# muelea/tuch

Hardware: AMD Instinct MI355X
Metric: SMPLify-DC fit iters/sec at batch 64 (higher is better)
Workload: dtype f32; 1 GPU; configs[1] extended to the full stage-2 step: batch=64/GPU SMPL forward + contact_fitting_loss (L_P/L_C push/pull, winding inside test, segment filter, r2r) + backward + Adam, V=6890 F=13776, float32; bodies_per_gpu=64, global_batch=64, launch=hipGraph replay of the whole step

## Files before the change

include/tuch_amd.h:

```cpp
#ifndef TUCH_AMD_H
#define TUCH_AMD_H

#include <stddef.h>
#include <stdint.h>

#ifdef __cplusplus
extern "C" {
#endif

const char* tuch_last_error(void);
int tuch_abi_version(void);

typedef struct tuch_contact_model tuch_contact_model;


int tuch_batch_pairwise_dist(const float* x, const float* y, int B, int Nx, int Ny, int squared,
                             float* P, void* stream);

int tuch_batch_pairwise_dist_bwd(const float* x, const float* y, const float* grad_P, int B, int Nx, int Ny,
                                 int squared, float* grad_x, float* grad_y, void* stream);

int tuch_solid_angles_bwd(const float* points, const float* triangles, const float* grad_out, const float* grad_w,
                          int B, int Q, int F, float* grad_points, float* grad_triangles, void* stream);

// ... 103 lines not shown
int tuch_contact_model_get_option(const tuch_contact_model* model, const char* name, int* value);
int tuch_contact_model_canary_hits(const tuch_contact_model* model, int* hits_host, int reset);
int tuch_contact_model_canary_selftest(const tuch_contact_model* model, void* workspace, size_t workspace_bytes, void* stream);
const uint64_t* tuch_contact_model_mask_bits(const tuch_contact_model* model);
const uint64_t* tuch_contact_model_tree_mask_bits(const tuch_contact_model* model);
int tuch_contact_model_info(const tuch_contact_model* model, int* V, int* F, int* num_segments,
                            int* seg_q_total, int* num_pairs);
int tuch_contact_model_strips(const tuch_contact_model* model, int* stream_len, int* num_strips,
                              int32_t* vidx_host, float* sign_host);

int tuch_winding_tree_work(const tuch_contact_model* model, const float* verts, int B, void* workspace,
                           size_t workspace_bytes, unsigned long long* out_host, void* stream);

int tuch_ray_work(const tuch_contact_model* model, const float* verts, int B, void* workspace,
                  size_t workspace_bytes, unsigned long long* out_host, void* stream);
int tuch_contact_model_tree_order(const tuch_contact_model* model, int32_t* qperm_host, int32_t* face_leaf_host);

size_t tuch_v2v_model_workspace_bytes(const tuch_contact_model* model, int B);
size_t tuch_v2v_hint_bytes(const tuch_contact_model* model, int B);
enum { TUCH_V2V_LEAVE_ROOM = 1, TUCH_V2V_NEAR_FINAL = 2 };
int tuch_v2v_min_model(const tuch_contact_model* model, const float* verts, int B, float* min_d2, int32_t* argmin,
                       void* hint_inout, void* workspace, size_t workspace_bytes, int flags, void* zero, size_t zero_bytes,
                       void* stream);

typedef struct tuch_cluster_tree tuch_cluster_tree;
int tuch_cluster_tree_build(int V, int F, const int32_t* faces, int leaf_faces, tuch_cluster_tree** out);
void tuch_cluster_tree_free(tuch_cluster_tree* tree);
int tuch_cluster_tree_info(const tuch_cluster_tree* tree, int* num_nodes, int* exact_len, int* stream_len,
                           int* num_qblocks, int* num_frontiers, int* frontier_total);
int tuch_cluster_tree_export(const tuch_cluster_tree* tree, int32_t* nodes, int32_t* vidx, float* sign,
// ... 128 lines not shown
```

tuch_amd/_C.py:

```python
from __future__ import annotations

import contextlib
import ctypes
import os
from ctypes import POINTER, c_char_p, c_float, c_int, c_size_t, c_uint, c_void_p

import torch

_HERE = os.path.dirname(os.path.abspath(__file__))
LIB_PATH = os.environ.get('TUCH_AMD_LIB') or os.path.join(_HERE, 'libtuch_amd.so')
_lib = None

ABI_VERSION = 2

_SIGNATURES = {
    'tuch_last_error': (c_char_p, []),
    'tuch_abi_version': (c_int, []),
    'tuch_batch_pairwise_dist': (c_int, [c_void_p, c_void_p, c_int, c_int, c_int, c_int, c_void_p, c_void_p]),
    'tuch_batch_pairwise_dist_bwd': (c_int, [c_void_p, c_void_p, c_void_p, c_int, c_int, c_int, c_int, c_void_p, c_void_p,
                                             c_void_p]),
    'tuch_solid_angles_bwd': (c_int, [c_void_p, c_void_p, c_void_p, c_void_p, c_int, c_int, c_int, c_void_p, c_void_p, c_void_p]),
    'tuch_solid_angles': (c_int, [c_void_p, c_void_p, c_int, c_int, c_int, c_void_p, c_void_p]),
    'tuch_gather_triangles': (c_int, [c_void_p, c_void_p, c_int, c_int, c_int, c_void_p, c_void_p]),
    'tuch_winding_workspace_bytes': (c_size_t, [c_int, c_int, c_int]),
# ... 56 lines not shown
    'tuch_estimate_translation': (c_int, [c_void_p, c_void_p, c_void_p, c_int, c_int, c_float, c_float, c_void_p, c_void_p]),
    'tuch_rotmat_to_angle_axis': (c_int, [c_void_p, c_int, c_int, c_void_p, c_void_p]),
    'tuch_winding_tree_work': (c_int, [c_void_p, c_void_p, c_int, c_void_p, c_size_t, c_void_p, c_void_p]),
    'tuch_hd_model_create': (c_int, [POINTER(c_void_p), c_void_p, c_int, c_void_p, c_void_p, c_void_p]),
    'tuch_hd_model_create_k': (c_int, [POINTER(c_void_p), c_void_p, c_int, c_int, c_void_p, c_void_p, c_void_p]),
    'tuch_hd_model_destroy': (None, [c_void_p]),
    'tuch_hd_model_info': (c_int, [c_void_p, POINTER(c_int), c_void_p]),
    'tuch_hd_contact_saved_bytes': (c_size_t, [c_void_p, c_int]),
    'tuch_hd_contact_workspace_bytes': (c_size_t, [c_void_p, c_int]),
    'tuch_hd_contact_fwd': (c_int, [c_void_p] * 6 + [c_int, c_float, c_float, c_void_p, c_void_p, c_size_t, c_void_p, c_size_t,
                                    c_void_p]),
    'tuch_hd_contact_bwd': (c_int, [c_void_p, c_void_p, c_void_p, c_int, c_void_p, c_void_p, c_size_t, c_void_p]),
    'tuch_hd_contact_selection': (c_int, [c_void_p, c_void_p, c_int, c_void_p, c_void_p]),
    'tuch_hd_contact_details': (c_int, [c_void_p, c_void_p, c_int, c_void_p, c_void_p]),
    'tuch_ray_work': (c_int, [c_void_p, c_void_p, c_int, c_void_p, c_size_t, c_void_p, c_void_p]),
    'tuch_contact_model_tree_order': (c_int, [c_void_p, c_void_p, c_void_p]),
    'tuch_v2v_model_workspace_bytes': (c_size_t, [c_void_p, c_int]),
    'tuch_v2v_hint_bytes': (c_size_t, [c_void_p, c_int]),
    'tuch_v2v_min_model': (c_int, [c_void_p, c_void_p, c_int, c_void_p, c_void_p, c_void_p, c_void_p, c_size_t, c_int,
                                   c_void_p, c_size_t, c_void_p]),
    'tuch_exterior_workspace_bytes': (c_size_t, [c_void_p, c_int]),
    'tuch_exterior_flags': (c_int, [c_void_p, c_void_p, c_int, c_int, c_float, c_void_p, c_void_p, c_void_p,
                                    c_void_p, c_void_p, c_size_t, c_void_p]),
    'tuch_winding_points_workspace_bytes': (c_size_t, [c_void_p, c_int, c_int]),
    'tuch_winding_points': (c_int, [c_void_p, c_void_p, c_void_p, c_void_p, c_int, c_int, c_float, c_void_p, c_void_p,
                                    c_void_p, c_size_t, c_void_p]),
    'tuch_closest_point_workspace_bytes': (c_size_t, [c_void_p, c_int, c_int]),
    'tuch_closest_point': (c_int, [c_void_p, c_void_p, c_void_p, c_void_p, c_int, c_int, c_void_p, c_void_p, c_void_p,
                                   c_void_p, c_size_t, c_void_p]),
    'tuch_closest_point_bwd': (c_int, [c_void_p] * 6 + [c_int, c_int] + [c_void_p] * 4),
# ... 106 lines not shown
```

tuch_amd/csrc/model.h:

```cpp
#pragma once
#include "common.h"
#include <vector>

enum { kNodeCapOff, kNodeCapLen, kNodeExactOff, kNodeExactLen, kNodeSkip, kNodeChild0, kNodeChild1, kNodeFaces, kNodeWords };
struct tuch_rows { int first, count; };
struct tuch_cluster_tree {
    int V = 0, F = 0, num_nodes = 0, exact_len = 0, stream_len = 0, num_qblocks = 0, num_heights = 0;
    std::vector<int32_t> nodes;
    std::vector<int32_t> vidx;
    std::vector<float> sign;
    std::vector<int32_t> qperm;
    std::vector<int32_t> height_off, height_nodes;
    std::vector<int32_t> frontier_off, frontier_nodes;
    std::vector<int32_t> launch_order;
    std::vector<int32_t> ancestors;
    std::vector<int32_t> rows;
    std::vector<int32_t> face_leaf;

    int node(int i, int field) const { return nodes[(size_t)i * kNodeWords + field]; }
    int skip(int i) const { return node(i, kNodeSkip); }
    int child0(int i) const { return node(i, kNodeChild0); }
    int child1(int i) const { return node(i, kNodeChild1); }
    bool is_leaf(int i) const { return child0(i) < 0; }
    int num_faces(int i) const { return node(i, kNodeFaces); }
// ... 4 lines not shown
};

bool tuch_cluster_tree_build_impl(int V, int F, const int32_t* faces, int leaf_faces, tuch_cluster_tree& t);
void tuch_build_strips(const int32_t* faces, int F, std::vector<int32_t>& vidx, std::vector<float>& sign,
                       int* num_strips);

struct tuch_contact_model;

struct tuch_options {
    int winding_ray = 1;
    int winding_tree = 1;
    int winding_strips = 1;
    int tree_waves = 32768;
    int ray_pair_cap = 16;
    int ray_waves = 32768;
    int v2v_tree = 1;
    int v2v_waves = 0;
    int v2v_flat = 2;
    int v2v_pairs = 24;
    int v2v_lds = -1;
    int seg_splits = 16;
    int seg_assist = 1;
    int seg_fused = 1;
    int canary = 0;
    int hd_search = 1;
    int hd_search_waves = 4;
    int hd_overlap = 1;
};
void tuch_options_from_env(tuch_options* o);

// ... 6 lines not shown
size_t tuch_ray_workspace_bytes(const tuch_contact_model* m, int B, int Q);
int tuch_ray_exterior_verts(const tuch_contact_model* m, const float* verts, int B, float thresh, uint8_t* exterior,
                            float* w, void* workspace, hipStream_t s, unsigned long long* stats_host,
                            uint8_t* exterior_copy = nullptr);
const int32_t* tuch_ray_segment_counts(const tuch_contact_model* m, int B, const void* workspace);
void tuch_ray_segment_prepare(const tuch_contact_model* m, const float* verts, const float* caps, int assisted, int B,
                              float* seg_entries, hipStream_t s);
bool tuch_ray_segment_fused_available(const tuch_contact_model* m);
int tuch_ray_segment_flags_one(const tuch_contact_model* m, const float* verts, const uint8_t* body_flags,
                               const int32_t* leaf_counts, int B, float thresh, uint8_t* exterior, hipStream_t s);
int tuch_ray_segment_flags(const tuch_contact_model* m, const float* verts, const float* caps, const int32_t* seg_count,
                           const int32_t* seg_list, const int32_t* leaf_counts, int B, int nsplit, float thresh, float* seg_tris,
                           int32_t* seg_partial, float* seg_w, uint8_t* seg_ext, uint8_t* exterior, hipStream_t s);
int tuch_ray_exterior_points(const tuch_contact_model* m, const float* verts, const float* points, const int32_t* counts,
                             int B, int Q, float thresh, uint8_t* exterior, float* w, void* workspace, hipStream_t s);

int tuch_v2v_min_indexed_seeded(const float* points, const int32_t* vertex_ids, const int32_t* offsets,
                                const int32_t* counts, const float* seed_best, const int32_t* seed_arg,
                                const int32_t* all_masked_arg, const uint64_t* geomask_bits, int B, int V,
                                int max_points_per_body, float* min_d2, int32_t* argmin, void* workspace, hipStream_t s);
extern "C" size_t tuch_v2v_min_indexed_workspace_bytes(int B, int max_points_per_body);
size_t tuch_hd_search_workspace_bytes(int B, int max_points_per_body);
int tuch_hd_search(const float* points, const int32_t* vertex_ids, const int32_t* offsets, const int32_t* counts,
                   const int32_t* all_masked_arg, const uint64_t* geomask_bits, int B, int V, int max_points_per_body,
                   float* min_d2, int32_t* argmin, void* workspace, hipStream_t s, int waves);
extern "C" size_t tuch_winding_points_workspace_bytes(const tuch_contact_model* m, int B, int Q);
extern "C" int tuch_winding_points(const tuch_contact_model* m, const float* verts, const float* points,
                                   const int32_t* counts, int B, int Q, float thresh, float* w,
                                   uint8_t* exterior, void* workspace, size_t workspace_bytes, void* stream);

// ... 73 lines not shown
```

tuch_amd/csrc/model.hip:

```cpp
#include "model.h"
#include <stdarg.h>
#include <stdio.h>
#include <stdlib.h>
#include <string.h>
#include <algorithm>
#include <vector>
#include <unordered_map>

extern "C" int tuch_geomask_words(int V);

namespace {

struct Segments {
    int count, num_caps;
    const int32_t *q_off, *q_vidx, *f_off, *faces;
};

struct SegmentLists {
    std::vector<int32_t> link_off{0}, links;
    std::vector<int32_t> ray_off{0}, ray_ent;
    std::vector<int32_t> elem_mask;
};

void debug_note(const char* fmt, ...)
// ... 431 lines not shown
        build_leaf_assist_tables(m, tree, faces, sg, lists);
    }
    if (num_regions > 0) build_region_tables(m, geomask, num_regions, region_off, region_vidx, num_pairs, pairs);
    if (!tree.sign.empty()) build_sign_words(m, tree, lists.elem_mask);
    const int rc = m->tables.rc;
    *out = rc == TUCH_OK ? m : nullptr;
    if (rc != TUCH_OK) tuch_contact_model_destroy(m);
    return rc;
}

namespace {
struct OptionName { const char* name; int tuch_options::*field; };
const OptionName kOptions[] = {
    {"winding_ray", &tuch_options::winding_ray}, {"winding_tree", &tuch_options::winding_tree},
    {"winding_strips", &tuch_options::winding_strips}, {"tree_waves", &tuch_options::tree_waves},
    {"ray_pair_cap", &tuch_options::ray_pair_cap}, {"ray_waves", &tuch_options::ray_waves},
    {"v2v_tree", &tuch_options::v2v_tree}, {"v2v_flat", &tuch_options::v2v_flat}, {"v2v_pairs", &tuch_options::v2v_pairs}, {"v2v_waves", &tuch_options::v2v_waves}, {"v2v_lds", &tuch_options::v2v_lds},
    {"seg_splits", &tuch_options::seg_splits}, {"seg_assist", &tuch_options::seg_assist}, {"seg_fused", &tuch_options::seg_fused},
    {"canary", &tuch_options::canary}, {"hd_search", &tuch_options::hd_search}, {"hd_search_waves", &tuch_options::hd_search_waves}, {"hd_overlap", &tuch_options::hd_overlap},
};
}

void tuch_options_from_env(tuch_options* o)
{
    for (const OptionName& k : kOptions) {
        char env[64] = "TUCH_";
        size_t n = strlen(env);
        for (const char* c = k.name; *c && n + 1 < sizeof(env); ++c) env[n++] = (char)toupper((unsigned char)*c);
        env[n] = 0;
        const char* e = getenv(env);
        if (e && *e) o->*(k.field) = atoi(e);
// ... 82 lines not shown
```

tuch_amd/csrc/ray_winding.hip:

```cpp
#include "common.h"
#include "model.h"
#include "workspace.h"
#include "tree_device.h"
#include <stdlib.h>

#pragma clang fp contract(off)

namespace {

constexpr float kPi = 3.14159265358979323846f;
constexpr int kBlock = 256;
constexpr int kRayQueries = 64;
constexpr float kShearX = 0.3217f, kShearY = 0.4331f;
constexpr float kFanX = 0.8191f, kFanY = 0.3467f, kFanZ = 0.4571f;
constexpr int kSlabs = 9;
constexpr int kSlabStride = 10;
constexpr int kNearSlabs = 13;

struct RayElem { float x, y, z, sign; };

__device__ __forceinline__ float shear_x(float x, float z) { return __builtin_fmaf(-kShearX, z, x); }
__device__ __forceinline__ float shear_y(float y, float z) { return __builtin_fmaf(-kShearY, z, y); }

__global__ __launch_bounds__(kBlock) void ray_stream_kernel(
// ... 94 lines not shown
        for (int p = Lexact + (int)threadIdx.x; p < T; p += kBoundsBlock)
            boxes[(size_t)b * T + p] = make_float4(__builtin_inff(), -__builtin_inff(), __builtin_inff(), -__builtin_inff());
    auto posed = [&](int p) {
        RayElem e;
        if (kPose) {
            const float* c = verts + ((size_t)b * V + vidx[p]) * 3;
            e.x = shear_x(c[0], c[2]); e.y = shear_y(c[1], c[2]); e.z = c[2]; e.sign = sign[p];
        } else {
            e = st[p];
        }
        return e;
    };
    float lo[kSlabs], nhi[kSlabs];
#pragma unroll
    for (int k = 0; k < kSlabs; ++k) { lo[k] = 3.0e38f; nhi[k] = 3.0e38f; }
    for (int p = sub; p < len; p += 16) {
        const RayElem e = posed(off + p);
        if (kPose) stream_out[(size_t)b * T + off + p] = e;
        boxes[(size_t)b * T + off + p] = ray_elem_box(posed(off + max(p - 2, 0)), posed(off + max(p - 1, 0)), e);
        float pr[kSlabs];
        slab_project(e.x, e.y, e.z, pr);
#pragma unroll
        for (int k = 0; k < kSlabs; ++k) { lo[k] = fminf(lo[k], pr[k]); nhi[k] = fminf(nhi[k], -pr[k]); }
    }
#pragma unroll
    for (int k = 0; k < kSlabs; ++k) { lo[k] = row_min(lo[k]); nhi[k] = row_min(nhi[k]); }
    if (real && sub == 0) {
        const int L = height_off[1] - height_off[0], leaf = i - height_off[0];
        float lo_p[kSlabs], hi_p[kSlabs];
#pragma unroll
        for (int k = 0; k < kSlabs; ++k) {
            const float hi = -nhi[k];
            const float pad = 4e-7f * fmaxf(fabsf(lo[k]), fabsf(hi)) + 1e-9f;
            lo_p[k] = lo[k] - pad;
            hi_p[k] = hi + pad;
        }
        float c[3];
        if (kPose) {
// ... 438 lines not shown
    }
    const int total_pairs = sp[kTilesBlock - 1], total_tiles = st[kTilesBlock - 1];
    const bool overflow = total_pairs > cap || total_tiles > max_tiles;
    if (t == 0) body[b] = RayBody{overflow ? fallback_tiles : total_tiles, overflow ? 1 : 0};
    if (overflow) return;
    int off = sp[t] - pairs, tile = st[t] - ntile;
    RayTile* out = tiles + (size_t)b * max_tiles;
    for (int l = l0; l < l1; ++l) {
        leaf_off[(size_t)b * num_leaves + l] = off;
        const TreeNode nd = nodes[leaf_nodes[l]];
        for (int k = 0; k < cnt[l]; k += 64) out[tile++] = RayTile{nd.ex_off, nd.ex_len, off + k, min(64, cnt[l] - k)};
        off += cnt[l];
    }
}

__global__ __launch_bounds__(64) void ray_fill_kernel(
    const RayEntry* __restrict__ lists, const int32_t* __restrict__ list_len, const RayBody* __restrict__ body,
    const int32_t* __restrict__ leaf_off, int num_leaves, int qblocks, int cap, int32_t* __restrict__ leaf_fill,
    int32_t* __restrict__ pairs)
{
    const int qb = blockIdx.x, b = blockIdx.y, lane = threadIdx.x;
    if (body[b].overflow) return;
    const int cnt = list_len[(size_t)b * qblocks + qb];
    const RayEntry* list = lists + ((size_t)b * qblocks + qb) * num_leaves;
    int32_t* out = pairs + (size_t)b * cap;
    for (int base = 0; base < cnt; base += 64) {
        const int j = base + lane;
        RayEntry e = RayEntry{0, 0, 0u, 0u};
        int dst = 0;
        if (j < cnt) {
            e = list[j];
            const int n = __builtin_popcount(e.mask_lo) + __builtin_popcount(e.mask_hi);
            dst = leaf_off[(size_t)b * num_leaves + e.leaf] + atomicAdd(&leaf_fill[(size_t)b * num_leaves + e.leaf], n);
        }
        const int m = min(64, cnt - base);
        for (int k = 0; k < m; ++k) {
            const uint32_t lo = __builtin_amdgcn_readlane(e.mask_lo, k), hi = __builtin_amdgcn_readlane(e.mask_hi, k);
            const int d = __builtin_amdgcn_readlane(dst, k);
            const unsigned long long mask = ((unsigned long long)hi << 32) | lo;
            if ((mask >> lane) & 1ull)
                out[d + __builtin_popcountll(mask & ((1ull << lane) - 1ull))] = qb * kRayQueries + lane;
        }
    }
}

constexpr int kTilesFillBlock = 64, kFillSplit = 64, kFillMaxBlocks = 2048;
__device__ __forceinline__ int wave_inclusive_scan(int v, int lane)
{
#pragma unroll
    for (int d = 1; d < 64; d <<= 1) {
        const int up = __shfl_up(v, d, 64);
        if (lane >= d) v += up;
    }
    return v;
}
__global__ __launch_bounds__(kTilesFillBlock) void ray_tiles_fill_kernel(
    const int32_t* __restrict__ leaf_cnt, const TreeNode* __restrict__ nodes, const int32_t* __restrict__ leaf_nodes,
    int num_leaves, int cap, int max_tiles, int fallback_tiles, RayTile* __restrict__ tiles, RayBody* __restrict__ body,
    const RayEntry* __restrict__ lists, const int32_t* __restrict__ list_len, int qblocks, int32_t* __restrict__ leaf_fill,
    int32_t* __restrict__ pairs, int list_stride)
{
    __builtin_amdgcn_s_setprio(3);
    extern __shared__ int32_t dyn[];
    int32_t* off_s = dyn;
    int32_t* tile_s = dyn + num_leaves;
    int32_t* blk = dyn + 2 * num_leaves;
    const int b = blockIdx.x, lane = threadIdx.x;
    const int per = (num_leaves + 63) / 64;
    const int l0 = min(lane * per, num_leaves), l1 = min(l0 + per, num_leaves);
    const int perq = (qblocks + 63) / 64;
    const int q0 = min(lane * perq, qblocks), q1 = min(q0 + perq, qblocks);
    const int32_t* cnt = leaf_cnt + (size_t)b * num_leaves;
    const int32_t* len = list_len + (size_t)b * qblocks;
    int npairs = 0, ntile = 0, nent = 0;
    for (int l = l0; l < l1; ++l) { const int c = cnt[l]; npairs += c; ntile += (c + 63) >> 6; }
    for (int q = q0; q < q1; ++q) nent += len[q];
    const int sp = wave_inclusive_scan(npairs, lane), st = wave_inclusive_scan(ntile, lane), sq = wave_inclusive_scan(nent, lane);
    const int total_pairs = __builtin_amdgcn_readlane(sp, 63), total_tiles = __builtin_amdgcn_readlane(st, 63);
    const int total = __builtin_amdgcn_readlane(sq, 63);
    const bool overflow = total_pairs > cap || total_tiles > max_tiles;
    if (lane == 0 && blockIdx.y == 0) body[b] = RayBody{overflow ? fallback_tiles : total_tiles, overflow ? 1 : 0};
    if (overflow) return;
    {
        int off = sp - npairs, tile = st - ntile;
        for (int l = l0; l < l1; ++l) {
            const int c = cnt[l];
            off_s[l] = off;
            tile_s[l] = tile;
            off += c;
            tile += (c + 63) >> 6;
        }
        int ent = sq - nent;
        for (int q = q0; q < q1; ++q) { blk[q] = ent; ent += len[q]; }
        if (lane == 0) blk[qblocks] = total;
    }
    __syncthreads();
    for (int l = (int)blockIdx.y + (int)gridDim.y * lane; l < num_leaves; l += (int)gridDim.y * 64) {
        const TreeNode nd = nodes[leaf_nodes[l]];
        const int ex_off = nd.ex_off, ex_len = nd.ex_len;
        const int c = cnt[l], off = off_s[l];
        RayTile* out = tiles + (size_t)b * max_tiles + tile_s[l];
        for (int k = 0; k < c; k += 64) *out++ = RayTile{ex_off, ex_len, off + k, min(64, c - k)};
    }
    int32_t* fill = leaf_fill + (size_t)b * num_leaves;
    int32_t* out = pairs + (size_t)b * cap;
    for (int base = (int)blockIdx.y * 64; base < total; base += (int)gridDim.y * 64) {
        const int g = base + lane;
        RayEntry e = RayEntry{0, 0, 0u, 0u};
        int dst = 0, qb = 0;
        if (g < total) {
            int lo = 0, hi = qblocks;
            while (hi - lo > 1) {
                const int mid = (lo + hi) >> 1;
                if (blk[mid] <= g) lo = mid; else hi = mid;
            }
            qb = lo;
            e = lists[((size_t)b * qblocks + qb) * list_stride + (g - blk[qb])];
            dst = off_s[e.leaf] + atomicAdd(&fill[e.leaf], __builtin_popcount(e.mask_lo) + __builtin_popcount(e.mask_hi));
        }
        const int m = min(64, total - base);
        for (int k = 0; k < m; ++k) {
            const uint32_t lo = __builtin_amdgcn_readlane(e.mask_lo, k), hi = __builtin_amdgcn_readlane(e.mask_hi, k);
            const int d = __builtin_amdgcn_readlane(dst, k), q = __builtin_amdgcn_readlane(qb, k);
            const unsigned long long mask = ((unsigned long long)hi << 32) | lo;
            if ((mask >> lane) & 1ull)
                out[d + __builtin_popcountll(mask & ((1ull << lane) - 1ull))] = q * kRayQueries + lane;
        }
    }
}

template <bool kVerts, bool kCount, bool kSeg>
__global__ __launch_bounds__(64) void ray_leaf_kernel(
    const float* __restrict__ pts, const RayElem* __restrict__ stream, const float4* __restrict__ boxes,
    const RayTile* __restrict__ tiles, const RayBody* __restrict__ body, const int32_t* __restrict__ pairs, const RayEntry* __restrict__ lists,
    const int32_t* __restrict__ list_len, const TreeNode* __restrict__ nodes, int num_leaves,
    const int32_t* __restrict__ qperm, const int32_t* __restrict__ counts, int Q, int T, int qblocks, int num_bodies,
    int cap, int max_tiles, int32_t* __restrict__ count, unsigned long long* __restrict__ stats,
    const int32_t* __restrict__ vmask, int32_t* __restrict__ seg_count)
{
    const int lane = threadIdx.x;
    struct Work { int b, off, len, slot, qmask; bool active; float qx, qy, qz; float4 pre; RayElem pre_el; };
    int b_cur = blockIdx.x, base = 0, g = blockIdx.y;
// ... 827 lines not shown
                           (const int32_t*)m->tree_vidx, (const float*)m->tree_sign_word, m->V, m->tree_exact_len, st,
                           (uint4*)(ws + l.zeroed), l.zeroed_bytes / sizeof(uint4), (float4*)(ws + l.boxes));
        return;
    }
    hipLaunchKernelGGL(ray_stream_kernel, dim3(ceil_div(l.T, kBlock), B), dim3(kBlock), 0, s, verts,
                       (const int32_t*)m->tree_vidx, (const float*)m->tree_sign_word, m->V, m->tree_exact_len, l.T, st,
                       (uint4*)(ws + l.zeroed), l.zeroed_bytes / sizeof(uint4));
    hipLaunchKernelGGL(ray_leaf_bounds_kernel<false>, dim3(ceil_div(m->tree_leaves, kBoundsBlock / 16), B), dim3(kBoundsBlock), 0, s,
                       (const RayElem*)st, l.T, (const TreeNode*)m->tree_node, m->tree_nodes,
                       (const int32_t*)m->tree_height_off, (const int32_t*)m->tree_height_nodes, bounds,
                       (const float*)nullptr, (const int32_t*)nullptr, (const float*)nullptr, 0, m->tree_exact_len, (RayElem*)nullptr,
                       (uint4*)nullptr, (size_t)0, (float4*)(ws + l.boxes));
}

template <bool kVerts>
static int launch_ray_counts(const tuch_contact_model* m, const RayLayout& l, const float* verts, const float* queries,
                             const int32_t* counts, int B, int Q, char* ws, hipStream_t s, unsigned long long* stats)
{
    launch_ray_boxes(m, l, verts, B, ws, s, kVerts);
    const int L = m->tree_leaves;
    const TreeNode* nodes = (const TreeNode*)m->tree_node;
    const int32_t* leaf_nodes = (const int32_t*)m->tree_height_nodes;
    const int32_t* qperm = kVerts ? (const int32_t*)m->tree_qperm : nullptr;
    RayEntry* lists = (RayEntry*)(ws + l.lists);
    int32_t* list_len = (int32_t*)(ws + l.list_len);
    int32_t* leaf_cnt = (int32_t*)(ws + l.leaf_cnt);
    int32_t* leaf_off = (int32_t*)(ws + l.leaf_off);
    RayTile* tiles = (RayTile*)(ws + l.tiles);
    RayBody* body = (RayBody*)(ws + l.body);
    int32_t* pairs = (int32_t*)(ws + l.pairs);
    if ((long)l.qblocks * B <= 2048)
        hipLaunchKernelGGL((ray_near_kernel<kVerts, 4>), dim3(l.qblocks, B), dim3(256), 0, s, queries, nodes,
                           (const float*)(ws + l.bounds), m->tree_nodes, L, qperm, counts, Q, l.qblocks, lists, list_len,
                           leaf_cnt, stats);
    else
        hipLaunchKernelGGL((ray_near_kernel<kVerts, 1>), dim3(l.qblocks, B), dim3(64), 0, s, queries, nodes,
                           (const float*)(ws + l.bounds), m->tree_nodes, L, qperm, counts, Q, l.qblocks, lists, list_len,
                           leaf_cnt, stats);
    const size_t tf_lds = (2 * (size_t)L + l.qblocks + 1) * sizeof(int32_t);
    if (l.qblocks <= kFillMaxBlocks && tf_lds <= 48u * 1024)
        hipLaunchKernelGGL(ray_tiles_fill_kernel, dim3(B, std::min(256, std::max(kFillSplit, 2048 / B))), dim3(kTilesFillBlock), tf_lds, s, (const int32_t*)leaf_cnt,
                           nodes, leaf_nodes, L, l.cap, l.max_tiles, l.qblocks * kFallbackChunks, tiles, body,
                           (const RayEntry*)lists, (const int32_t*)list_len, l.qblocks, (int32_t*)(ws + l.leaf_fill), pairs, L);
    else {
    hipLaunchKernelGGL(ray_tiles_kernel, dim3(B), dim3(kTilesBlock), 0, s, (const int32_t*)leaf_cnt, nodes, leaf_nodes, L, l.cap,
                       l.max_tiles, l.qblocks * kFallbackChunks, leaf_off, tiles, body);
    hipLaunchKernelGGL(ray_fill_kernel, dim3(l.qblocks, B), dim3(64), 0, s, (const RayEntry*)lists, (const int32_t*)list_len,
                       (const RayBody*)body, (const int32_t*)leaf_off, L, l.qblocks, l.cap, (int32_t*)(ws + l.leaf_fill), pairs);
    }
    const dim3 grid(l.columns, l.workers);
    const bool seg = kVerts && m->seg_elem_mask;
    const int32_t* vmask = (const int32_t*)m->seg_vmask;
    int32_t* seg_count = (int32_t*)(ws + l.seg_count);
#define TUCH_LAUNCH_RAY_LEAF(COUNT, SEG)                                                                                      \
    hipLaunchKernelGGL((ray_leaf_kernel<kVerts, COUNT, SEG>), grid, dim3(64), 0, s, queries, (const RayElem*)(ws + l.stream),  \
                       (const float4*)(ws + l.boxes), (const RayTile*)tiles, (const RayBody*)body, (const int32_t*)pairs, (const RayEntry*)lists,            \
                       (const int32_t*)list_len, nodes, L, qperm, counts, Q, l.T, l.qblocks, B, l.cap, l.max_tiles,           \
                       (int32_t*)(ws + l.count), stats, vmask, seg_count)
    if (stats) {
        if (seg) TUCH_LAUNCH_RAY_LEAF(true, kVerts); else TUCH_LAUNCH_RAY_LEAF(true, false);
    } else {
        if (seg) TUCH_LAUNCH_RAY_LEAF(false, kVerts); else TUCH_LAUNCH_RAY_LEAF(false, false);
    }
#undef TUCH_LAUNCH_RAY_LEAF
// ... 31 lines not shown
{
    if (!m->seg_elem_mask) return nullptr;
    return (const int32_t*)((const char*)workspace + full_layout(m, B, m->V, true).seg_count);
}

int tuch_ray_exterior_points(const tuch_contact_model* m, const float* verts, const float* points, const int32_t* counts,
                             int B, int Q, float thresh, uint8_t* exterior, float* w, void* workspace, hipStream_t s)
{
    const RayLayout l = full_layout(m, B, Q, false);
    char* ws = (char*)workspace;
    const int rc = launch_ray_counts<false>(m, l, verts, points, counts, B, Q, ws, s, nullptr);
    if (rc != TUCH_OK) return rc;
    hipLaunchKernelGGL(ray_finalize_points_kernel, dim3(ceil_div(Q, kBlock), B), dim3(kBlock), 0, s,
                       (const int32_t*)(ws + l.count), counts, Q, l.qblocks * kRayQueries, thresh, w, exterior);
    return tuch_check_launch("tuch_ray_exterior_points");
}

void tuch_ray_segment_prepare(const tuch_contact_model* m, const float* verts, const float* caps, int assisted, int B,
                              float* seg_entries, hipStream_t s)
{
    const bool as = assisted && m->seg_cap_off;
    const int E = as ? m->seg_cap_total : m->seg_ray_total;
    hipLaunchKernelGGL(segment_shear_entries_kernel, dim3(ceil_div(E > 0 ? E : 1, kBlock), B), dim3(kBlock), 0, s,
                       verts, caps, (const int32_t*)(as ? m->seg_cap_ent : m->seg_ray_ent), m->V, m->num_caps, E, seg_entries);
}

int tuch_ray_segment_flags(const tuch_contact_model* m, const float* verts, const float* caps, const int32_t* seg_count,
                           const int32_t* seg_list, const int32_t* leaf_counts, int B, int nsplit, float thresh,
                           float* seg_entries, int32_t* seg_partial, float* seg_w, uint8_t* seg_ext, uint8_t* exterior,
                           hipStream_t s)
// ... 25 lines not shown
```

tuch_amd/csrc/winding.hip:

```cpp
#include "common.h"
#include "model.h"
#include "workspace.h"
#include "tree_device.h"
#include <stdlib.h>

namespace {

constexpr float kPi = 3.14159265358979323846f;
constexpr float kHalfPi = 1.57079632679489661923f;
constexpr int kBlock = 256;
constexpr int kQueriesPerLane = 2;
constexpr int kQueriesPerBlock = kBlock * kQueriesPerLane;
constexpr int kStripBlock = 128;
constexpr int kStripQueries = kStripBlock * kQueriesPerLane;

__device__ __forceinline__ v2f atan_poly(v2f t)
{
    const v2f s = t * t;
    v2f p = splat2(0.0024567253421992064f);
    p = fma2(p, s, splat2(-0.014401361346244812f));
    p = fma2(p, s, splat2(0.03978123143315315f));
    p = fma2(p, s, splat2(-0.07234857976436615f));
    p = fma2(p, s, splat2(0.10498946160078049f));
    p = fma2(p, s, splat2(-0.14161229133605957f));
// ... 957 lines not shown

extern "C" int tuch_ray_work(const tuch_contact_model* m, const float* verts, int B, void* workspace,
                             size_t workspace_bytes, unsigned long long* out_host, void* stream)
{
    TUCH_REQUIRE(m && verts && out_host, "tuch_ray_work: null pointer");
    TUCH_REQUIRE(tuch_ray_available(m), "tuch_ray_work: the model has no cluster tree / vertex rings");
    TUCH_REQUIRE(B > 0 && B <= 65535, "tuch_ray_work: bad batch %d", B);
    const ExteriorLayout l = exterior_layout(m, B);
    if (!workspace || workspace_bytes < l.total) {
        tuch_set_error("tuch_ray_work: workspace %zu < %zu bytes", workspace_bytes, l.total);
        return TUCH_ERR_WORKSPACE;
    }
    return tuch_ray_exterior_verts(m, verts, B, 0.99f, nullptr, nullptr, (char*)workspace + l.ray, (hipStream_t)stream, out_host);
}

struct PointsLayout { size_t stream, bounds, partial, total; int frontier, nsub, qblocks; };

static PointsLayout points_layout(const tuch_contact_model* m, int B, int Q)
{
    PointsLayout l;
    l.qblocks = ceil_div(Q, kTreeQueries);
    int f = 0;
    while (f + 1 < m->tree_num_frontiers &&
           (long)B * l.qblocks * (m->tree_frontier_off_host[f + 1] - m->tree_frontier_off_host[f]) < 65536L) ++f;
    l.frontier = f;
    l.nsub = m->tree_frontier_off_host[f + 1] - m->tree_frontier_off_host[f];
    size_t o = 0;
    l.stream = tuch_ws_take(o, (size_t)B * (m->tree_stream_len + 3) * sizeof(StreamElem));
    l.bounds = tuch_ws_take(o, (size_t)B * m->tree_nodes * 2 * kSlabStride * sizeof(float));
    l.partial = tuch_ws_take(o, (size_t)B * l.nsub * l.qblocks * kTreeQueries * sizeof(float));
// ... 78 lines not shown
```

tuch_amd/ops.py:

```python
from __future__ import annotations

import contextlib
import ctypes
import os
import weakref
from typing import Dict, List, NamedTuple, Optional, Sequence, Tuple

import numpy as np
import torch
from torch.autograd.function import once_differentiable

from . import _C, backward_pass
from .backward_pass import backward_scalar

MODE_SMPLIFY = 0
MODE_TRAIN = 1


def _f32(t: torch.Tensor) -> torch.Tensor:
    if t.dtype is torch.float32 and t.is_contiguous():
        return t.detach()
    return t.detach().to(torch.float32).contiguous()


# ... 1060 lines not shown
        return dict(leaf_elements=int(out[0]), cap_elements=int(out[1]), wavefronts=int(out[2]),
                    flat_stream_elements=int(out[3]), queries_per_step=64,
                    query_blocks=-(-self.num_verts // 128) * 2 * b)

    def ray_work(self, verts: torch.Tensor) -> dict:
        verts = _f32(verts)
        b = verts.shape[0]
        L = _C.lib()
        nbytes = L.tuch_exterior_workspace_bytes(self._handle, b)
        ws = _workspace(nbytes, verts.device)
        out = (ctypes.c_ulonglong * 4)()
        _C.check(L.tuch_ray_work(self._handle, _C.ptr(verts), b, _C.ptr(ws), nbytes, out, _C.stream()))
        return dict(elements=int(out[0]), wavefronts=int(out[3]), queries_per_step=64,
                    lanes_inside_leaf_slabs=int(out[1]) / max(int(out[2]), 1))

    def exterior_flags(self, verts: torch.Tensor, apply_segments: bool = True, thresh: float = 0.99,
                       return_details: bool = False):
        verts = _f32(verts)
        b = verts.shape[0]
        assert verts.shape[1] == self.num_verts
        L = _C.lib()
        ext = torch.empty(b, self.num_verts, dtype=torch.uint8, device=verts.device)
        w = torch.empty(b, self.num_verts, dtype=torch.float32, device=verts.device) if return_details else None
        seg_w = seg_e = None
        if return_details and self.num_segments:
            seg_w = torch.empty(b, self.seg_q_total, dtype=torch.float32, device=verts.device)
            seg_e = torch.empty(b, self.seg_q_total, dtype=torch.uint8, device=verts.device)
        nbytes = L.tuch_exterior_workspace_bytes(self._handle, b)
        ws = _workspace(nbytes, verts.device)
        _C.check(L.tuch_exterior_flags(self._handle, _C.ptr(verts), b, int(apply_segments), float(thresh),
# ... 415 lines not shown
```

Baseline: 159,200 body-fit iterations/s.

## Parallelize ray pair fill with LDS staging and reuse neighbor elements via DPP

The ray pair fill used to loop serially over the 64 list entries in a wave with readlane broadcasts. It now does a wave prefix scan over per-entry pair counts, stages the masks and offsets in LDS, and has each lane write one output pair using a binary search plus a k-th-set-bit select. The box kernel now gets the two previous stream elements from neighbouring lanes through DPP moves instead of reloading and re-posing them. The tiles-fill kernel also keeps small per-lane count arrays in registers. A debug check entry point is added to validate pairs and boxes, and it adds extra syncthreads and LDS use to the fill path.

```diff
diff --git a/include/tuch_amd.h b/include/tuch_amd.h
--- a/include/tuch_amd.h
+++ b/include/tuch_amd.h
@@ -141,6 +141,8 @@
 
 int tuch_ray_work(const tuch_contact_model* model, const float* verts, int B, void* workspace,
                   size_t workspace_bytes, unsigned long long* out_host, void* stream);
+int tuch_ray_fill_check(const tuch_contact_model* model, const float* verts, const float* points, const int32_t* counts,
+                        int B, int Q, void* workspace, size_t workspace_bytes, unsigned long long* out_host, void* stream);
 int tuch_contact_model_tree_order(const tuch_contact_model* model, int32_t* qperm_host, int32_t* face_leaf_host);
 
 size_t tuch_v2v_model_workspace_bytes(const tuch_contact_model* model, int B);
diff --git a/tuch_amd/_C.py b/tuch_amd/_C.py
--- a/tuch_amd/_C.py
+++ b/tuch_amd/_C.py
@@ -94,6 +94,7 @@
     'tuch_hd_contact_selection': (c_int, [c_void_p, c_void_p, c_int, c_void_p, c_void_p]),
     'tuch_hd_contact_details': (c_int, [c_void_p, c_void_p, c_int, c_void_p, c_void_p]),
     'tuch_ray_work': (c_int, [c_void_p, c_void_p, c_int, c_void_p, c_size_t, c_void_p, c_void_p]),
+    'tuch_ray_fill_check': (c_int, [c_void_p, c_void_p, c_void_p, c_void_p, c_int, c_int, c_void_p, c_size_t, c_void_p, c_void_p]),
     'tuch_contact_model_tree_order': (c_int, [c_void_p, c_void_p, c_void_p]),
     'tuch_v2v_model_workspace_bytes': (c_size_t, [c_void_p, c_int]),
     'tuch_v2v_hint_bytes': (c_size_t, [c_void_p, c_int]),
diff --git a/tuch_amd/csrc/model.h b/tuch_amd/csrc/model.h
--- a/tuch_amd/csrc/model.h
+++ b/tuch_amd/csrc/model.h
@@ -42,6 +42,7 @@
     int tree_waves = 32768;
     int ray_pair_cap = 16;
     int ray_waves = 32768;
+    int ray_fill_split = 0;
     int v2v_tree = 1;
     int v2v_waves = 0;
     int v2v_flat = 2;
@@ -78,6 +79,8 @@
                            int32_t* seg_partial, float* seg_w, uint8_t* seg_ext, uint8_t* exterior, hipStream_t s);
 int tuch_ray_exterior_points(const tuch_contact_model* m, const float* verts, const float* points, const int32_t* counts,
                              int B, int Q, float thresh, uint8_t* exterior, float* w, void* workspace, hipStream_t s);
+int tuch_ray_fill_check_impl(const tuch_contact_model* m, const float* verts, const float* points, const int32_t* counts,
+                             int B, int Q, void* workspace, hipStream_t s, unsigned long long* out_host);
 
 int tuch_v2v_min_indexed_seeded(const float* points, const int32_t* vertex_ids, const int32_t* offsets,
                                 const int32_t* counts, const float* seed_best, const int32_t* seed_arg,
diff --git a/tuch_amd/csrc/model.hip b/tuch_amd/csrc/model.hip
--- a/tuch_amd/csrc/model.hip
+++ b/tuch_amd/csrc/model.hip
@@ -469,7 +469,7 @@
 const OptionName kOptions[] = {
     {"winding_ray", &tuch_options::winding_ray}, {"winding_tree", &tuch_options::winding_tree},
     {"winding_strips", &tuch_options::winding_strips}, {"tree_waves", &tuch_options::tree_waves},
-    {"ray_pair_cap", &tuch_options::ray_pair_cap}, {"ray_waves", &tuch_options::ray_waves},
+    {"ray_pair_cap", &tuch_options::ray_pair_cap}, {"ray_waves", &tuch_options::ray_waves}, {"ray_fill_split", &tuch_options::ray_fill_split},
     {"v2v_tree", &tuch_options::v2v_tree}, {"v2v_flat", &tuch_options::v2v_flat}, {"v2v_pairs", &tuch_options::v2v_pairs}, {"v2v_waves", &tuch_options::v2v_waves}, {"v2v_lds", &tuch_options::v2v_lds},
     {"seg_splits", &tuch_options::seg_splits}, {"seg_assist", &tuch_options::seg_assist}, {"seg_fused", &tuch_options::seg_fused},
     {"canary", &tuch_options::canary}, {"hd_search", &tuch_options::hd_search}, {"hd_search_waves", &tuch_options::hd_search_waves}, {"hd_overlap", &tuch_options::hd_overlap},
diff --git a/tuch_amd/csrc/ray_fill_util.h b/tuch_amd/csrc/ray_fill_util.h
--- /dev/null
+++ b/tuch_amd/csrc/ray_fill_util.h
@@ -0,0 +1,39 @@
+#pragma once
+#include <stdint.h>
+
+#if defined(__HIPCC__) || defined(__CUDACC__)
+#define TUCH_FILL_FN __host__ __device__ inline __attribute__((always_inline))
+#else
+#define TUCH_FILL_FN inline
+#endif
+
+TUCH_FILL_FN int tuch_kth_set_bit64(uint32_t lo, uint32_t hi, int k)
+{
+    const int nlo = __builtin_popcount(lo);
+    const bool upper = k >= nlo;
+    uint32_t w = upper ? hi : lo;
+    k -= upper ? nlo : 0;
+    int pos = upper ? 32 : 0;
+    int c = __builtin_popcount(w & 0xffffu);
+    if (k >= c) { k -= c; pos += 16; w >>= 16; }
+    c = __builtin_popcount(w & 0xffu);
+    if (k >= c) { k -= c; pos += 8; w >>= 8; }
+    c = __builtin_popcount(w & 0xfu);
+    if (k >= c) { k -= c; pos += 4; w >>= 4; }
+    c = __builtin_popcount(w & 0x3u);
+    if (k >= c) { k -= c; pos += 2; w >>= 2; }
+    c = (int)(w & 1u);
+    if (k >= c) pos += 1;
+    return pos;
+}
+
+TUCH_FILL_FN int tuch_prefix_interval64(const int32_t* ex, int r, int* start)
+{
+    int j = 0, base = 0;
+    for (int step = 32; step >= 1; step >>= 1) {
+        const int v = ex[j + step];
+        if (v <= r) { j += step; base = v; }
+    }
+    *start = base;
+    return j;
+}
diff --git a/tuch_amd/csrc/ray_winding.hip b/tuch_amd/csrc/ray_winding.hip
--- a/tuch_amd/csrc/ray_winding.hip
+++ b/tuch_amd/csrc/ray_winding.hip
@@ -2,6 +2,7 @@
 #include "model.h"
 #include "workspace.h"
 #include "tree_device.h"
+#include "ray_fill_util.h"
 #include <stdlib.h>
 
 #pragma clang fp contract(off)
@@ -132,14 +133,28 @@
     float lo[kSlabs], nhi[kSlabs];
 #pragma unroll
     for (int k = 0; k < kSlabs; ++k) { lo[k] = 3.0e38f; nhi[k] = 3.0e38f; }
-    for (int p = sub; p < len; p += 16) {
-        const RayElem e = posed(off + p);
-        if (kPose) stream_out[(size_t)b * T + off + p] = e;
-        boxes[(size_t)b * T + off + p] = ray_elem_box(posed(off + max(p - 2, 0)), posed(off + max(p - 1, 0)), e);
-        float pr[kSlabs];
-        slab_project(e.x, e.y, e.z, pr);
-#pragma unroll
-        for (int k = 0; k < kSlabs; ++k) { lo[k] = fminf(lo[k], pr[k]); nhi[k] = fminf(nhi[k], -pr[k]); }
+    float prev_x = 0.f, prev_y = 0.f;
+    for (int base = 0; base < len; base += 16) {
+        const int p = base + sub;
+        const bool live = p < len;
+        RayElem e = RayElem{0.f, 0.f, 0.f, 0.f};
+        if (live) {
+            e = posed(off + p);
+            if (kPose) stream_out[(size_t)b * T + off + p] = e;
+        }
+        RayElem p1 = RayElem{dpp_move<0x121>(sub == 15 ? prev_x : e.x), dpp_move<0x121>(sub == 15 ? prev_y : e.y), 0.f, 0.f};
+        RayElem p2 = RayElem{dpp_move<0x122>(sub >= 14 ? prev_x : e.x), dpp_move<0x122>(sub >= 14 ? prev_y : e.y), 0.f, 0.f};
+        if (p == 0) p1 = e;
+        if (p < 2) p2 = p1;
+        prev_x = e.x;
+        prev_y = e.y;
+        if (live) {
+            boxes[(size_t)b * T + off + p] = ray_elem_box(p2, p1, e);
+            float pr[kSlabs];
+            slab_project(e.x, e.y, e.z, pr);
+#pragma unroll
+            for (int k = 0; k < kSlabs; ++k) { lo[k] = fminf(lo[k], pr[k]); nhi[k] = fminf(nhi[k], -pr[k]); }
+        }
     }
 #pragma unroll
     for (int k = 0; k < kSlabs; ++k) { lo[k] = row_min(lo[k]); nhi[k] = row_min(nhi[k]); }
@@ -608,6 +623,45 @@
     }
 }
 
+__device__ __forceinline__ int wave_inclusive_scan(int v, int lane)
+{
+#pragma unroll
+    for (int d = 1; d < 64; d <<= 1) {
+        const int up = __shfl_up(v, d, 64);
+        if (lane >= d) v += up;
+    }
+    return v;
+}
+
+struct RayFillStage { int32_t ex[64]; uint4 ent[64]; };
+template <int kWide>
+__device__ __forceinline__ void ray_fill_rays(const RayFillStage& st, int r0, int R, int lane, int32_t* __restrict__ out)
+{
+    int j[kWide], start[kWide];
+#pragma unroll
+    for (int u = 0; u < kWide; ++u) j[u] = tuch_prefix_interval64(st.ex, r0 + 64 * u + lane, &start[u]);
+#pragma unroll
+    for (int u = 0; u < kWide; ++u) {
+        const int r = r0 + 64 * u + lane;
+        const uint4 e = st.ent[j[u]];
+        if (r < R) out[(int)e.z + r] = (int)e.w * kRayQueries + tuch_kth_set_bit64(e.x, e.y, r - start[u]);
+    }
+}
+__device__ __forceinline__ void ray_fill_trip(RayFillStage& st, uint32_t mask_lo, uint32_t mask_hi, int n, int dst, int qb,
+                                              int lane, int32_t* __restrict__ out)
+{
+    const int inc = wave_inclusive_scan(n, lane);
+    const int R = __builtin_amdgcn_readlane(inc, 63);
+    __syncthreads();
+    st.ex[lane] = inc - n;
+    st.ent[lane] = make_uint4(mask_lo, mask_hi, (uint32_t)(dst - (inc - n)), (uint32_t)qb);
+    __syncthreads();
+    int r0 = 0;
+    for (; R - r0 > 128; r0 += 256) ray_fill_rays<4>(st, r0, R, lane, out);
+    if (R - r0 > 64) ray_fill_rays<2>(st, r0, R, lane, out);
+    else if (R - r0 > 0) ray_fill_rays<1>(st, r0, R, lane, out);
+}
+
 __global__ __launch_bounds__(64) void ray_fill_kernel(
     const RayEntry* __restrict__ lists, const int32_t* __restrict__ list_len, const RayBody* __restrict__ body,
     const int32_t* __restrict__ leaf_off, int num_leaves, int qblocks, int cap, int32_t* __restrict__ leaf_fill,
@@ -618,36 +672,21 @@
     const int cnt = list_len[(size_t)b * qblocks + qb];
     const RayEntry* list = lists + ((size_t)b * qblocks + qb) * num_leaves;
     int32_t* out = pairs + (size_t)b * cap;
+    __shared__ RayFillStage stage;
     for (int base = 0; base < cnt; base += 64) {
         const int j = base + lane;
         RayEntry e = RayEntry{0, 0, 0u, 0u};
-        int dst = 0;
+        int dst = 0, n = 0;
         if (j < cnt) {
             e = list[j];
-            const int n = __builtin_popcount(e.mask_lo) + __builtin_popcount(e.mask_hi);
+            n = __builtin_popcount(e.mask_lo) + __builtin_popcount(e.mask_hi);
             dst = leaf_off[(size_t)b * num_leaves + e.leaf] + atomicAdd(&leaf_fill[(size_t)b * num_leaves + e.leaf], n);
         }
-        const int m = min(64, cnt - base);
-        for (int k = 0; k < m; ++k) {
-            const uint32_t lo = __builtin_amdgcn_readlane(e.mask_lo, k), hi = __builtin_amdgcn_readlane(e.mask_hi, k);
-            const int d = __builtin_amdgcn_readlane(dst, k);
-            const unsigned long long mask = ((unsigned long long)hi << 32) | lo;
-            if ((mask >> lane) & 1ull)
-                out[d + __builtin_popcountll(mask & ((1ull << lane) - 1ull))] = qb * kRayQueries + lane;
-        }
+        ray_fill_trip(stage, e.mask_lo, e.mask_hi, n, dst, qb, lane, out);
     }
 }
 
 constexpr int kTilesFillBlock = 64, kFillSplit = 64, kFillMaxBlocks = 2048;
-__device__ __forceinline__ int wave_inclusive_scan(int v, int lane)
-{
-#pragma unroll
-    for (int d = 1; d < 64; d <<= 1) {
-        const int up = __shfl_up(v, d, 64);
-        if (lane >= d) v += up;
-    }
-    return v;
-}
 __global__ __launch_bounds__(kTilesFillBlock) void ray_tiles_fill_kernel(
     const int32_t* __restrict__ leaf_cnt, const TreeNode* __restrict__ nodes, const int32_t* __restrict__ leaf_nodes,
     int num_leaves, int cap, int max_tiles, int fallback_tiles, RayTile* __restrict__ tiles, RayBody* __restrict__ body,
@@ -666,9 +705,40 @@
     const int q0 = min(lane * perq, qblocks), q1 = min(q0 + perq, qblocks);
     const int32_t* cnt = leaf_cnt + (size_t)b * num_leaves;
     const int32_t* len = list_len + (size_t)b * qblocks;
+    constexpr int kPer = 8, kPerQ = 4;
+    const bool few = per <= kPer, fewq = perq <= kPerQ;
+    int creg[kPer], qreg[kPerQ];
+    if (few) {
+#pragma unroll
+        for (int i = 0; i < kPer; ++i) creg[i] = cnt[min(l0 + i, num_leaves - 1)];
+    }
+    if (fewq) {
+#pragma unroll
+        for (int i = 0; i < kPerQ; ++i) qreg[i] = len[min(q0 + i, qblocks - 1)];
+    }
+    const int tl = (int)blockIdx.y + (int)gridDim.y * lane;
+    const TreeNode& tnode = nodes[leaf_nodes[min(tl, num_leaves - 1)]];
+    const int t_off = tnode.ex_off, t_len = tnode.ex_len, t_cnt = cnt[min(tl, num_leaves - 1)];
     int npairs = 0, ntile = 0, nent = 0;
-    for (int l = l0; l < l1; ++l) { const int c = cnt[l]; npairs += c; ntile += (c + 63) >> 6; }
-    for (int q = q0; q < q1; ++q) nent += len[q];
+    if (few) {
+#pragma unroll
+        for (int i = 0; i < kPer; ++i) {
+            if (l0 + i >= l1) creg[i] = 0;
+            npairs += creg[i];
+            ntile += (creg[i] + 63) >> 6;
+        }
+    } else {
+        for (int l = l0; l < l1; ++l) { const int c = cnt[l]; npairs += c; ntile += (c + 63) >> 6; }
+    }
+    if (fewq) {
+#pragma unroll
+        for (int i = 0; i < kPerQ; ++i) {
+            if (q0 + i >= q1) qreg[i] = 0;
+            nent += qreg[i];
+        }
+    } else {
+        for (int q = q0; q < q1; ++q) nent += len[q];
+    }
     const int sp = wave_inclusive_scan(npairs, lane), st = wave_inclusive_scan(ntile, lane), sq = wave_inclusive_scan(nent, lane);
     const int total_pairs = __builtin_amdgcn_readlane(sp, 63), total_tiles = __builtin_amdgcn_readlane(st, 63);
     const int total = __builtin_amdgcn_readlane(sq, 63);
@@ -677,31 +747,52 @@
     if (overflow) return;
     {
         int off = sp - npairs, tile = st - ntile;
-        for (int l = l0; l < l1; ++l) {
-            const int c = cnt[l];
-            off_s[l] = off;
-            tile_s[l] = tile;
-            off += c;
-            tile += (c + 63) >> 6;
+        if (few) {
+#pragma unroll
+            for (int i = 0; i < kPer; ++i)
+                if (l0 + i < l1) {
+                    off_s[l0 + i] = off;
+                    tile_s[l0 + i] = tile;
+                    off += creg[i];
+                    tile += (creg[i] + 63) >> 6;
+                }
+        } else {
+            for (int l = l0; l < l1; ++l) {
+                const int c = cnt[l];
+                off_s[l] = off;
+                tile_s[l] = tile;
+                off += c;
+                tile += (c + 63) >> 6;
+            }
         }
         int ent = sq - nent;
-        for (int q = q0; q < q1; ++q) { blk[q] = ent; ent += len[q]; }
+        if (fewq) {
+#pragma unroll
+            for (int i = 0; i < kPerQ; ++i)
+                if (q0 + i < q1) { blk[q0 + i] = ent; ent += qreg[i]; }
+        } else {
+            for (int q = q0; q < q1; ++q) { blk[q] = ent; ent += len[q]; }
+        }
         if (lane == 0) blk[qblocks] = total;
     }
     __syncthreads();
-    for (int l = (int)blockIdx.y + (int)gridDim.y * lane; l < num_leaves; l += (int)gridDim.y * 64) {
-        const TreeNode nd = nodes[leaf_nodes[l]];
-        const int ex_off = nd.ex_off, ex_len = nd.ex_len;
-        const int c = cnt[l], off = off_s[l];
+    for (int l = tl; l < num_leaves; l += (int)gridDim.y * 64) {
+        int ex_off = t_off, ex_len = t_len, c = t_cnt;
+        if (l != tl) {
+            const TreeNode& nd = nodes[leaf_nodes[l]];
+            ex_off = nd.ex_off; ex_len = nd.ex_len; c = cnt[l];
+        }
+        const int off = off_s[l];
         RayTile* out = tiles + (size_t)b * max_tiles + tile_s[l];
         for (int k = 0; k < c; k += 64) *out++ = RayTile{ex_off, ex_len, off + k, min(64, c - k)};
     }
     int32_t* fill = leaf_fill + (size_t)b * num_leaves;
     int32_t* out = pairs + (size_t)b * cap;
+    __shared__ RayFillStage stage;
     for (int base = (int)blockIdx.y * 64; base < total; base += (int)gridDim.y * 64) {
         const int g = base + lane;
         RayEntry e = RayEntry{0, 0, 0u, 0u};
-        int dst = 0, qb = 0;
+        int dst = 0, qb = 0, n = 0;
         if (g < total) {
             int lo = 0, hi = qblocks;
             while (hi - lo > 1) {
@@ -710,16 +801,10 @@
             }
             qb = lo;
             e = lists[((size_t)b * qblocks + qb) * list_stride + (g - blk[qb])];
-            dst = off_s[e.leaf] + atomicAdd(&fill[e.leaf], __builtin_popcount(e.mask_lo) + __builtin_popcount(e.mask_hi));
-        }
-        const int m = min(64, total - base);
-        for (int k = 0; k < m; ++k) {
-            const uint32_t lo = __builtin_amdgcn_readlane(e.mask_lo, k), hi = __builtin_amdgcn_readlane(e.mask_hi, k);
-            const int d = __builtin_amdgcn_readlane(dst, k), q = __builtin_amdgcn_readlane(qb, k);
-            const unsigned long long mask = ((unsigned long long)hi << 32) | lo;
-            if ((mask >> lane) & 1ull)
-                out[d + __builtin_popcountll(mask & ((1ull << lane) - 1ull))] = q * kRayQueries + lane;
-        }
+            n = __builtin_popcount(e.mask_lo) + __builtin_popcount(e.mask_hi);
+            dst = off_s[e.leaf] + atomicAdd(&fill[e.leaf], n);
+        }
+        ray_fill_trip(stage, e.mask_lo, e.mask_hi, n, dst, qb, lane, out);
     }
 }
 
@@ -1577,7 +1662,7 @@
 }
 
 template <bool kVerts>
-static int launch_ray_counts(const tuch_contact_model* m, const RayLayout& l, const float* verts, const float* queries,
+static void launch_ray_lists(const tuch_contact_model* m, const RayLayout& l, const float* verts, const float* queries,
                              const int32_t* counts, int B, int Q, char* ws, hipStream_t s, unsigned long long* stats)
 {
     launch_ray_boxes(m, l, verts, B, ws, s, kVerts);
@@ -1602,7 +1687,9 @@
                            leaf_cnt, stats);
     const size_t tf_lds = (2 * (size_t)L + l.qblocks + 1) * sizeof(int32_t);
     if (l.qblocks <= kFillMaxBlocks && tf_lds <= 48u * 1024)
-        hipLaunchKernelGGL(ray_tiles_fill_kernel, dim3(B, std::min(256, std::max(kFillSplit, 2048 / B))), dim3(kTilesFillBlock), tf_lds, s, (const int32_t*)leaf_cnt,
+        hipLaunchKernelGGL(ray_tiles_fill_kernel,
+                           dim3(B, m->opt.ray_fill_split > 0 ? std::min(m->opt.ray_fill_split, 1024) : std::min(256, std::max(kFillSplit, 2048 / B))),
+                           dim3(kTilesFillBlock), tf_lds, s, (const int32_t*)leaf_cnt,
                            nodes, leaf_nodes, L, l.cap, l.max_tiles, l.qblocks * kFallbackChunks, tiles, body,
                            (const RayEntry*)lists, (const int32_t*)list_len, l.qblocks, (int32_t*)(ws + l.leaf_fill), pairs, L);
     else {
@@ -1611,6 +1698,21 @@
     hipLaunchKernelGGL(ray_fill_kernel, dim3(l.qblocks, B), dim3(64), 0, s, (const RayEntry*)lists, (const int32_t*)list_len,
                        (const RayBody*)body, (const int32_t*)leaf_off, L, l.qblocks, l.cap, (int32_t*)(ws + l.leaf_fill), pairs);
     }
+}
+
+template <bool kVerts>
+static int launch_ray_counts(const tuch_contact_model* m, const RayLayout& l, const float* verts, const float* queries,
+                             const int32_t* counts, int B, int Q, char* ws, hipStream_t s, unsigned long long* stats)
+{
+    launch_ray_lists<kVerts>(m, l, verts, queries, counts, B, Q, ws, s, stats);
+    const int L = m->tree_leaves;
+    const TreeNode* nodes = (const TreeNode*)m->tree_node;
+    const int32_t* qperm = kVerts ? (const int32_t*)m->tree_qperm : nullptr;
+    const RayEntry* lists = (const RayEntry*)(ws + l.lists);
+    const int32_t* list_len = (const int32_t*)(ws + l.list_len);
+    const RayTile* tiles = (const RayTile*)(ws + l.tiles);
+    const RayBody* body = (const RayBody*)(ws + l.body);
+    const int32_t* pairs = (const int32_t*)(ws + l.pairs);
     const dim3 grid(l.columns, l.workers);
     const bool seg = kVerts && m->seg_elem_mask;
     const int32_t* vmask = (const int32_t*)m->seg_vmask;
@@ -1672,6 +1774,109 @@
     hipLaunchKernelGGL(ray_finalize_points_kernel, dim3(ceil_div(Q, kBlock), B), dim3(kBlock), 0, s,
                        (const int32_t*)(ws + l.count), counts, Q, l.qblocks * kRayQueries, thresh, w, exterior);
     return tuch_check_launch("tuch_ray_exterior_points");
+}
+
+namespace {
+
+__device__ __forceinline__ unsigned long long ray_pair_hash(int leaf, int slot)
+{
+    unsigned long long z = (((unsigned long long)(uint32_t)leaf << 32) | (uint32_t)slot) + 0x9e3779b97f4a7c15ull;
+    z = (z ^ (z >> 30)) * 0xbf58476d1ce4e5b9ull;
+    z = (z ^ (z >> 27)) * 0x94d049bb133111ebull;
+    return z ^ (z >> 31);
+}
+
+__global__ __launch_bounds__(64) void ray_check_pairs_kernel(
+    const RayEntry* __restrict__ lists, const int32_t* __restrict__ list_len, const RayBody* __restrict__ body,
+    const int32_t* __restrict__ leaf_cnt, const int32_t* __restrict__ leaf_fill, const int32_t* __restrict__ pairs,
+    int num_leaves, int qblocks, int cap, unsigned long long* __restrict__ out)
+{
+    const int leaf = blockIdx.x, b = blockIdx.y, lane = threadIdx.x;
+    if (body[b].overflow) return;
+    __shared__ unsigned long long acc[5];
+    if (lane < 5) acc[lane] = 0;
+    __syncthreads();
+    unsigned long long want_n = 0, want_sum = 0, entries = 0, off = 0;
+    for (int qb = lane; qb < qblocks; qb += 64) {
+        const int n = list_len[(size_t)b * qblocks + qb];
+        const RayEntry* list = lists + ((size_t)b * qblocks + qb) * num_leaves;
+        for (int j = 0; j < n; ++j) {
+            const RayEntry e = list[j];
+            if (e.leaf != leaf) continue;
+            ++entries;
+            const unsigned long long mask = ((unsigned long long)e.mask_hi << 32) | e.mask_lo;
+            for (int bit = 0; bit < 64; ++bit)
+                if ((mask >> bit) & 1ull) { ++want_n; want_sum += ray_pair_hash(leaf, qb * kRayQueries + bit); }
+        }
+    }
+    const int32_t* cnt = leaf_cnt + (size_t)b * num_leaves;
+    for (int l = lane; l < leaf; l += 64) off += (unsigned long long)cnt[l];
+    atomicAdd(&acc[0], want_n);
+    atomicAdd(&acc[1], want_sum);
+    atomicAdd(&acc[2], entries);
+    atomicAdd(&acc[3], off);
+    __syncthreads();
+    const long first = (long)acc[3], c = cnt[leaf];
+    unsigned long long got_sum = 0;
+    for (long i = lane; i < c; i += 64)
+        if (first + i < cap) got_sum += ray_pair_hash(leaf, pairs[(size_t)b * cap + first + i]);
+    atomicAdd(&acc[4], got_sum);
+    __syncthreads();
+    if (lane == 0) {
+        const bool bad = acc[0] != (unsigned long long)c || leaf_fill[(size_t)b * num_leaves + leaf] != c ||
+                         first + c > cap || acc[1] != acc[4];
+        if (bad) atomicAdd(out + 0, 1ull);
+        atomicAdd(out + 2, acc[0]);
+        atomicAdd(out + 3, acc[2]);
+    }
+}
+
+__global__ __launch_bounds__(64) void ray_check_boxes_kernel(
+    const float* __restrict__ verts, const int32_t* __restrict__ vidx, const float* __restrict__ sign, int V,
+    const TreeNode* __restrict__ nodes, const int32_t* __restrict__ leaf_nodes, const float4* __restrict__ boxes, int T,
+    unsigned long long* __restrict__ out)
+{
+    const int b = blockIdx.y;
+    const TreeNode nd = nodes[leaf_nodes[blockIdx.x]];
+    auto posed = [&](int p) {
+        const float* c = verts + ((size_t)b * V + vidx[p]) * 3;
+        return RayElem{shear_x(c[0], c[2]), shear_y(c[1], c[2]), c[2], sign[p]};
+    };
+    unsigned long long bad = 0;
+    for (int p = threadIdx.x; p < nd.ex_len; p += 64) {
+        const float4 want = ray_elem_box(posed(nd.ex_off + max(p - 2, 0)), posed(nd.ex_off + max(p - 1, 0)), posed(nd.ex_off + p));
+        const float4 got = boxes[(size_t)b * T + nd.ex_off + p];
+        bad += (__float_as_uint(want.x) != __float_as_uint(got.x)) + (__float_as_uint(want.y) != __float_as_uint(got.y)) +
+               (__float_as_uint(want.z) != __float_as_uint(got.z)) + (__float_as_uint(want.w) != __float_as_uint(got.w));
+    }
+    if (bad) atomicAdd(out + 1, bad);
+}
+
+}
+
+int tuch_ray_fill_check_impl(const tuch_contact_model* m, const float* verts, const float* points, const int32_t* counts,
+                             int B, int Q, void* workspace, hipStream_t s, unsigned long long* out_host)
+{
+    const bool vform = points == nullptr;
+    const RayLayout l = full_layout(m, B, vform ? m->V : Q, vform);
+    char* ws = (char*)workspace;
+    unsigned long long* out = (unsigned long long*)(ws + l.stats);
+    if (hipMemsetAsync(out, 0, 4 * sizeof(unsigned long long), s) != hipSuccess ||
+        hipMemsetAsync(ws + l.pairs, 0xff, (size_t)B * l.cap * sizeof(int32_t), s) != hipSuccess)
+        return TUCH_ERR_HIP;
+    if (vform) launch_ray_lists<true>(m, l, verts, verts, nullptr, B, m->V, ws, s, nullptr);
+    else launch_ray_lists<false>(m, l, verts, points, counts, B, Q, ws, s, nullptr);
+    const int L = m->tree_leaves;
+    hipLaunchKernelGGL(ray_check_pairs_kernel, dim3(L, B), dim3(64), 0, s, (const RayEntry*)(ws + l.lists),
+                       (const int32_t*)(ws + l.list_len), (const RayBody*)(ws + l.body), (const int32_t*)(ws + l.leaf_cnt),
+                       (const int32_t*)(ws + l.leaf_fill), (const int32_t*)(ws + l.pairs), L, l.qblocks, l.cap, out);
+    hipLaunchKernelGGL(ray_check_boxes_kernel, dim3(L, B), dim3(64), 0, s, verts, (const int32_t*)m->tree_vidx,
+                       (const float*)m->tree_sign_word, m->V, (const TreeNode*)m->tree_node,
+                       (const int32_t*)m->tree_height_nodes, (const float4*)(ws + l.boxes), l.T, out);
+    if (hipMemcpyAsync(out_host, out, 4 * sizeof(unsigned long long), hipMemcpyDeviceToHost, s) != hipSuccess ||
+        hipStreamSynchronize(s) != hipSuccess)
+        return TUCH_ERR_HIP;
+    return tuch_check_launch("tuch_ray_fill_check");
 }
 
 void tuch_ray_segment_prepare(const tuch_contact_model* m, const float* verts, const float* caps, int assisted, int B,
diff --git a/tuch_amd/csrc/winding.hip b/tuch_amd/csrc/winding.hip
--- a/tuch_amd/csrc/winding.hip
+++ b/tuch_amd/csrc/winding.hip
@@ -995,6 +995,28 @@
     return tuch_ray_exterior_verts(m, verts, B, 0.99f, nullptr, nullptr, (char*)workspace + l.ray, (hipStream_t)stream, out_host);
 }
 
+extern "C" int tuch_ray_fill_check(const tuch_contact_model* m, const float* verts, const float* points,
+                                   const int32_t* counts, int B, int Q, void* workspace, size_t workspace_bytes,
+                                   unsigned long long* out_host, void* stream)
+{
+    TUCH_REQUIRE(m && verts && out_host, "tuch_ray_fill_check: null pointer");
+    TUCH_REQUIRE(tuch_ray_available(m), "tuch_ray_fill_check: the model has no cluster tree / vertex rings");
+    TUCH_REQUIRE(B > 0 && B <= 65535 && (!points || Q > 0), "tuch_ray_fill_check: bad sizes B=%d Q=%d", B, Q);
+    size_t need = 0, at = 0;
+    if (points) {
+        need = tuch_winding_points_workspace_bytes(m, B, Q);
+    } else {
+        const ExteriorLayout l = exterior_layout(m, B);
+        need = l.total;
+        at = l.ray;
+    }
+    if (!workspace || workspace_bytes < need) {
+        tuch_set_error("tuch_ray_fill_check: workspace %zu < %zu bytes", workspace_bytes, need);
+        return TUCH_ERR_WORKSPACE;
+    }
+    return tuch_ray_fill_check_impl(m, verts, points, counts, B, Q, (char*)workspace + at, (hipStream_t)stream, out_host);
+}
+
 struct PointsLayout { size_t stream, bounds, partial, total; int frontier, nsub, qblocks; };
 
 static PointsLayout points_layout(const tuch_contact_model* m, int B, int Q)
diff --git a/tuch_amd/ops.py b/tuch_amd/ops.py
--- a/tuch_amd/ops.py
+++ b/tuch_amd/ops.py
@@ -1098,6 +1098,24 @@
         return dict(elements=int(out[0]), wavefronts=int(out[3]), queries_per_step=64,
                     lanes_inside_leaf_slabs=int(out[1]) / max(int(out[2]), 1))
 
+    def ray_fill_check(self, verts: torch.Tensor, points: Optional[torch.Tensor] = None,
+                       counts: Optional[torch.Tensor] = None) -> dict:
+        verts = _f32(verts)
+        b = verts.shape[0]
+        L = _C.lib()
+        pts, q = None, 0
+        if points is not None:
+            pts = _f32(points)
+            q = pts.shape[1]
+            nbytes = L.tuch_winding_points_workspace_bytes(self._handle, b, q)
+        else:
+            nbytes = L.tuch_exterior_workspace_bytes(self._handle, b)
+        ws = _workspace(nbytes, verts.device)
+        out = (ctypes.c_ulonglong * 4)()
+        _C.check(L.tuch_ray_fill_check(self._handle, _C.ptr(verts), _C.ptr(pts), _C.ptr(counts), b, q, _C.ptr(ws), nbytes, out,
+                                       _C.stream()))
+        return dict(bad_leaves=int(out[0]), bad_box_words=int(out[1]), pairs=int(out[2]), entries=int(out[3]))
+
     def exterior_flags(self, verts: torch.Tensor, apply_segments: bool = True, thresh: float = 0.99,
                        return_details: bool = False):
         verts = _f32(verts)
```

Measured after the change: 160,100 body-fit iterations/s (median of 3 runs). No clear change (+0.5%).
